# aantoine890/navierstokes

Hardware: AMD Instinct MI355X
Metric: fp64 CSR SpMV GFLOP/s & % HBM roofline @ nnz; 1/2/4/8 GPU (higher is better)
Workload: dtype f64

## Files before the change

include/mi355_spmv.h:

```cpp
#ifndef MI355_SPMV_H
#define MI355_SPMV_H

#ifdef __cplusplus
extern "C" {
#endif

#define MI355_SPMV_VERSION 501

enum {
    MI_OK = 0,
    MI_ERR_ARG = 1,
    MI_ERR_NODEVICE = 2,
    MI_ERR_HIP = 3,
    MI_ERR_ALLOC = 4,
    MI_ERR_UNSUPPORTED = 5,
    MI_ERR_STATE = 6
};

#define MI_MAX_POWERS 16

typedef struct mi_csr_s* mi_csr_t;
typedef struct mi_bcsr4_s* mi_bcsr4_t;
typedef struct mi_part_s* mi_part_t;
typedef void* mi_stream_t;

enum {
    MI_KERNEL_AUTO = 0,
    MI_KERNEL_STREAM = 1,
    MI_KERNEL_RING = 2,
    MI_KERNEL_ROWPAR = 3,
    MI_KERNEL_BCSR4 = 4,
    MI_KERNEL_MRING = 6,
    MI_KERNEL_SSTREAM = 7,
    MI_KERNEL_TILE = 5
};

int mi_version(void);
const char* mi_strerror(int status);
const char* mi_last_error(void);
int mi_device_count(int* count);
int mi_set_device(int device);
int mi_device_synchronize(void);
int mi_flush_cache(void);
int mi_flush_cache_async(mi_stream_t s);

int mi_csr_create(int n, int ncols, const int* ptrow, const int* indcol, const double* coef, mi_csr_t* out);
int mi_csr_create_mapped(int n, int ncols, const int* ptrow, const int* indcol, const double* coef,
                         const int* rowmap, mi_csr_t* out);
int mi_csr_destroy(mi_csr_t A);
int mi_csr_update_values(mi_csr_t A, const double* coef);
int mi_csr_update_values_dev(mi_csr_t A, const double* d_coef, mi_stream_t s);
int mi_csr_dims(mi_csr_t A, int* n, int* ncols, long long* nnz);
int mi_csr_reorder_info(mi_csr_t A, int* reordered, int* block, double* spread_before, double* spread_after,
                        double* us_natural, double* us_reordered);
int mi_csr_perm(mi_csr_t A, int* reordered, int* perm );
int mi_vec_to_internal_dev(mi_csr_t A, const double* d_x, double* d_x_int, mi_stream_t s);
int mi_vec_from_internal_dev(mi_csr_t A, const double* d_x_int, double* d_x, mi_stream_t s);
int mi_spmv_internal_dev(mi_csr_t A, const double* d_x_int, double* d_y_int, mi_stream_t s);
int mi_spmk_internal_dev(mi_csr_t A, int k, const double* d_x_int, double* const* d_y_int_out, mi_stream_t s);
int mi_reorder_probe(int n, const int* ptrow, const int* indcol, int* block, int* perm, double* spread_before,
                     double* spread_after);
int mi_csr_set_kernel(mi_csr_t A, int kernel_id);
int mi_csr_ring_info(mi_csr_t A, int* config_id, int* runs, int* runs_not_ringable, double* nnz_fraction_ringable);
int mi_csr_ring_shape_info(mi_csr_t A, int* blocks, int* lean, int* depth, double* us_aligned, double* us_unaligned);
int mi_csr_tune_info(mi_csr_t A, double* us_ring, double* us_stream);
int mi_csr_tune_detail(mi_csr_t A, double us[5], int* ring_nt, int* stream_nt);
int mi_ring_plan_probe(int n, const int* ptrow, const int* indcol, int config_id, int* nblk, int* runs,
                       int* runs_not_ringable, double* nnz_fraction_ringable, int* max_slot);
int mi_csr_tile_info(mi_csr_t A, int* built, int* nblk, double* unique_per_nnz, double us[2], int* nt);
int mi_tile_plan_probe(int n, const int* ptrow, const int* indcol, int threads, int* nblk, long long* distinct_total,
                       int* max_distinct, long long* nnz_listed);
int mi_csr_placement_info(mi_csr_t A, int* n_values, int* n_total, double* us, int cap);
int mi_vec_alloc_placed(mi_csr_t A, int nvec, int draws, double** d_vecs, double* us, int cap, int* n_us);
int mi_vec_free_placed(double* d_vec);
int mi_csr_sstream_info(mi_csr_t A, int* built, int* rounds, long long* steps, double* padding, double us[4], int* form);
int mi_sstream_plan_probe(int n, int ncols, const int* ptrow, const int* indcol, int* eligible, int* rounds, long long* steps, double* padding);
int mi_sstream_plan_probe_ex(int n, int ncols, const int* ptrow, const int* indcol, int shift, int ghost_lo, int ghost_hi, int* eligible, int* rounds,
                             long long* steps, double* padding, int* ghost_workgroups, int* rounds_min_max);
int mi_sstream_mw_plan_probe(int n, int ncols, const int* ptrow, const int* indcol, int shift, int* eligible, int* rounds, long long* steps, double* padding);
int mi_csr_mring_info(mi_csr_t A, int* built, int* runs, int* runs_not_served, double* nnz_fraction_served, double us[2], int* nt);
int mi_mring_plan_probe(int n, const int* ptrow, const int* indcol, int* nblk, int* runs, int* runs_not_served,
                        double* nnz_fraction_served, long long* window_restarts);
int mi_mring_plan_deal_probe(int n, const int* ptrow, const int* indcol, int* table_len, int* run_blocks, int cap);
int mi_ring_plan_lean(int n, const int* ptrow, const int* indcol, int config_id, int* lean);
#define MI_RING_CENSUS_LEN 62
int mi_ring_plan_census(int n, const int* ptrow, const int* indcol, int config_id, long long* counters, int cap);
#define MI_MRING_CENSUS_LEN 43
// ... 248 lines not shown
```

navierstokes_amd/csrc/capi_blas1.hip:

```cpp
#include "capi_internal.hpp"
#include "blas1_kernels.hpp"
#include "blas1_multi.hpp"
#include "gmres_kernels.hpp"

static std::map<std::pair<int, hipStream_t>, double*> g_ws;
constexpr size_t kWsMdot = 4 * (size_t)kMaxPartials;
constexpr size_t kWsDots2 = kWsMdot + (size_t)kMultiMax * kMaxPartials;
constexpr size_t kWsDoubles = kWsDots2 + kMultiMax + 8;

int get_ws(hipStream_t s, double** out)
{
    int dev = 0;
    HIP_TRY(hipGetDevice(&dev));
    std::lock_guard<std::mutex> lock(g_mu);
    double*& w = g_ws[std::make_pair(dev, s)];
    if (!w) HIP_TRY(hipMalloc(&w, sizeof(double) * kWsDoubles));
    *out = w;
    return MI_OK;
}

static bool blas1_nt(int n)
{
    static const int forced = getenv("MI355_BLAS1_NT") ? atoi(getenv("MI355_BLAS1_NT")) : -1;
    return forced >= 0 ? forced != 0 : n >= kBlas1NtMin;
}

static int red_geometry(int n, int* np, int* seg)
{
    long long s = ((long long)n + kMaxPartials - 1) / kMaxPartials;
    const int q = 2 * kRedWG;
    s = ((s + q - 1) / q) * q;
    if (s < q) s = q;
    *seg = (int)s;
    *np = (int)(((long long)n + s - 1) / s);
    if (*np < 1) *np = 1;
    return MI_OK;
// ... 565 lines not shown
    HIP_TRY(hipMemcpy(dots, dd, sizeof(double) * (size_t)m, hipMemcpyDeviceToHost));
    return MI_OK;
}

extern "C" int mi_maxpy(int n, int m, const double* coef, int negate, const double* const* basis, double* y)
{
    int rc = multi_check(n, m, basis, y);
    if (rc) return rc;
    CHECK_ARG(m == 0 || coef, "null coefficients");
    if ((rc = need_device())) return rc;
    if (m == 0 || n == 0) return MI_OK;
    Scratch S;
    std::vector<const double*> dv((size_t)m);
    double *dy = nullptr, *dc = nullptr;
    for (int j = 0; j < m; j++) {
        double* p = nullptr;
        if ((rc = S.up(basis[j], n, &p))) return rc;
        dv[j] = p;
    }
    if ((rc = S.up(y, n, &dy)) || (rc = S.up(coef, m, &dc))) return rc;
    if ((rc = mi_maxpy_dev(n, m, dc, negate, dv.data(), dy, nullptr, nullptr))) return rc;
    HIP_TRY(hipMemcpy(y, dy, sizeof(double) * (size_t)n, hipMemcpyDeviceToHost));
    return MI_OK;
}

int gather_perm(mi_csr_t A, const double* d_x, double* d_xp, hipStream_t s)
{
    if (A->reorder_block == 4 && (((uintptr_t)d_x | (uintptr_t)d_xp) & 15) == 0) {
        const int nn = A->n / 4;
        hipLaunchKernelGGL(gather_nodes_kernel, dim3(launch_grid(nn, 256, 4096)), dim3(256), 0, s, nn, A->d_iperm, d_x, d_xp);
        HIP_TRY(hipGetLastError());
        return MI_OK;
    }
    return mi_gather_dev(A->n, A->d_iperm, d_x, d_xp, (mi_stream_t)s);
}


__global__ __launch_bounds__(256) void scatter_kernel(int m, const int* __restrict__ idx, const double* __restrict__ src,
                                                      double* __restrict__ dst)
{
    const long long stride = (long long)gridDim.x * blockDim.x;
    for (long long i = (long long)blockIdx.x * blockDim.x + threadIdx.x; i < m; i += stride) dst[idx[i]] = src[i];
}

int scatter_perm(mi_csr_t A, const double* d_src, double* d_dst, hipStream_t s)
{
    hipLaunchKernelGGL(scatter_kernel, dim3(launch_grid(A->n, 256, 2048)), dim3(256), 0, s, A->n, A->d_iperm, d_src, d_dst);
    HIP_TRY(hipGetLastError());
    return MI_OK;
}
```

navierstokes_amd/csrc/capi_csr.hip:

```cpp
#include "capi_internal.hpp"
#include "reorder.hpp"
#include "mring_plan.hpp"
#include "tile_plan.hpp"

int get_table(mi_csr_t A, int nnzb, BlockTable** out)
{
    auto it = A->tables.find(nnzb);
    if (it == A->tables.end()) {
        std::vector<int> rows, ptrs;
        int row_align = A->nnz < 20000000 ? 64 : 1;
        if (const char* e = getenv("MI355_STREAM_ROW_ALIGN")) row_align = std::max(1, atoi(e));
        build_row_blocks(A->n, A->h_ptrow.data(), nnzb, 4 * kWG, rows, ptrs, row_align, 7);
        BlockTable T;
        T.nnzb = nnzb;
        T.nblk = (int)rows.size() - 1;
        std::vector<int2> h(rows.size());
        for (size_t i = 0; i < rows.size(); i++) h[i] = make_int2(rows[i], ptrs[i]);
        HIP_TRY(T.d_blk.upload(h));
        it = A->tables.emplace(nnzb, std::move(T)).first;
    }
    *out = &it->second;
    return MI_OK;
}

// ... 591 lines not shown
                    const int* rowmap, mi_csr_t* out, int ghost_lo, int ghost_hi, bool defer_placement)
{
    CHECK_ARG(out, "out is null");
    *out = nullptr;
    CsrInput in{n, ncols, ptrow, indcol, coef, rowmap, ghost_lo, ghost_hi};
    int rc = check_input(in);
    if (rc || (rc = need_device())) return rc;
    std::unique_ptr<mi_csr_s> owner(new (std::nothrow) mi_csr_s());
    mi_csr_t A = owner.get();
    if (!A) return fail(MI_ERR_ALLOC, "host allocation failed");
    A->n = n;
    A->ncols = ncols;
    A->nnz = in.nnz;
    A->ghost_lo = ghost_lo;
    A->ghost_hi = ghost_hi;
    A->h_ptrow.assign(ptrow, ptrow + n + 1);
    if ((rc = upload(A, in)) || (rc = plan_ring(A, in)) || (rc = plan_optional(A, in)) || (rc = attach_blocked(A, in))) return rc;
    load_defaults(A, in);
    const bool forced_kernel = apply_forced_kernel(A);
    if (!forced_kernel && in.nnz < kMeasureNnz && A->auto_kernel == MI_KERNEL_RING && !in.ghosts()) A->auto_kernel = MI_KERNEL_STREAM;
    if (!forced_kernel && !env_is("MI355_SPMV_AUTOTUNE", "0") && in.nnz >= kMeasureNnz && (rc = measure_at_create(A, in, defer_placement))) return rc;
    HIP_TRY(hipStreamSynchronize(nullptr));
    *out = owner.release();
    return MI_OK;
}

static int time_handle(mi_csr_t A, int warm, int timed, double* us)
{
    LaunchTimer tm;
    ScratchPair sp;
    int rc = sp.alloc((size_t)(A->ncols > 0 ? A->ncols : 1), (size_t)(A->n_out > 0 ? A->n_out : 1));
    if (rc || (rc = tm.init())) return rc;
    return time_on(tm, A, sp.x, sp.y, warm, timed, us);
}

static int maybe_reorder(mi_csr_t A, const int* ptrow, const int* indcol, const double* coef)
{
    const bool force = env_is("MI355_REORDER", "1");
    if (env_is("MI355_REORDER", "0")) return MI_OK;
    const int n = A->n;
    if (A->mapped || n != A->ncols || n < 8 || A->nnz == 0) return MI_OK;
    if (!force && (n < 100000 || resolve_kernel(A) == MI_KERNEL_RING || resolve_kernel(A) == MI_KERNEL_SSTREAM)) return MI_OK;
    const int block = csr_has_block4_pattern(n, ptrow, indcol) ? 4 : 1;
    const double nn = (double)n / block;
    const double spread = mean_column_distance(n, ptrow, indcol, block);
    A->spread_before = spread;
    if (!force && spread < 2.0 * std::pow(nn, 2.0 / 3.0)) return MI_OK;
    Reorder R;
    rcm_reorder(n, ptrow, indcol, block, R);
    A->reorder_block = block;
    A->spread_after = R.spread_after;
    if (!force && R.spread_after > 0.5 * spread) return MI_OK;
    std::vector<int> p2, c2, src_start;
    std::vector<double> v2;
    permute_csr(n, ptrow, indcol, coef, R, p2, c2, v2, src_start);
    mi_csr_t inner = nullptr;
    int rc = csr_create_impl(n, n, p2.data(), c2.data(), v2.data(), R.iperm.data(), &inner);
    if (rc) return rc;
    A->inner.reset(inner);
    HIP_TRY(A->d_iperm.alloc((size_t)n));
    HIP_TRY(A->d_src_start.alloc((size_t)n));
    HIP_TRY(A->d_xp.alloc((size_t)n));
    HIP_TRY(A->d_iperm.fill(R.iperm));
    HIP_TRY(A->d_src_start.fill(src_start));
    bool keep = true;
    if (!force && !env_is("MI355_SPMV_AUTOTUNE", "0")) {
        const int timed = A->nnz < 40000000 ? 12 : 6;
        (void)A->inner.own.release();
        rc = time_handle(A, 3, timed, &A->us_natural);
        A->inner.reset(inner);
        if (rc) return rc;
        if ((rc = time_handle(A, 3, timed, &A->us_reordered))) return rc;
        keep = A->us_reordered < 0.97 * A->us_natural;
    }
    if (!keep) {
        A->inner.reset(), A->d_iperm = {}, A->d_src_start = {}, A->d_xp = {};
        return MI_OK;
    }
    A->h_iperm = R.iperm;
    A->xp_claimed = false;
    A->d_ptrow = {}, A->d_indcol = {}, A->d_coef = {};
    A->drop_tables();
    A->ring = {}, A->tile = {}, A->mring = {}, A->ss = {}, A->blocked.reset();
    return MI_OK;
}

extern "C" int mi_csr_create(int n, int ncols, const int* ptrow, const int* indcol, const double* coef, mi_csr_t* out)
{
    int rc = csr_create_impl(n, ncols, ptrow, indcol, coef, nullptr, out, 0, 0, true);
    if (rc) return rc;
    if ((rc = maybe_reorder(*out, ptrow, indcol, coef)) || (!(*out)->inner && (rc = placement_draws(*out, nullptr, n == ncols))) ||
        (hipStreamSynchronize(nullptr) != hipSuccess && (rc = fail(MI_ERR_HIP, "mi_csr_create: synchronize")))) {
        mi_csr_destroy(*out);
        *out = nullptr;
    }
    return rc;
}

extern "C" int mi_reorder_probe(int n, const int* ptrow, const int* indcol, int* block, int* perm, double* spread_before,
                                double* spread_after)
{
    CHECK_ARG(n >= 0 && ptrow && (ptrow[n] == 0 || indcol), "bad argument");
    for (int i = 0; i < n; i++) {
        CHECK_ARG(ptrow[i] <= ptrow[i + 1], "ptrow must be non-decreasing");
        for (int k = ptrow[i]; k < ptrow[i + 1]; k++) CHECK_ARG(indcol[k] >= 0 && indcol[k] < n, "column index outside [0, n)");
    }
    const int b = csr_has_block4_pattern(n, ptrow, indcol) ? 4 : 1;
    Reorder R;
    rcm_reorder(n, ptrow, indcol, b, R);
    if (block) *block = b;
    if (perm)
        for (int i = 0; i < n; i++) perm[i] = R.perm[i];
    if (spread_before) *spread_before = R.spread_before;
    if (spread_after) *spread_after = R.spread_after;
    return MI_OK;
}

extern "C" int mi_csr_reorder_info(mi_csr_t A, int* reordered, int* block, double* spread_before, double* spread_after,
                                   double* us_natural, double* us_reordered)
{
    CHECK_ARG(A, "null handle");
    if (reordered) *reordered = A->inner ? 1 : 0;
    if (block) *block = A->reorder_block;
    if (spread_before) *spread_before = A->spread_before;
    if (spread_after) *spread_after = A->spread_after;
    if (us_natural) *us_natural = A->us_natural;
    if (us_reordered) *us_reordered = A->us_reordered;
    return MI_OK;
}

extern "C" int mi_csr_perm(mi_csr_t A, int* reordered, int* perm)
{
    CHECK_ARG(A, "null handle");
    if (reordered) *reordered = A->inner ? 1 : 0;
    if (perm) {
        if (A->inner) {
            CHECK_ARG((int)A->h_iperm.size() == A->n, "permutation not kept on this handle");
            for (int r = 0; r < A->n; r++) perm[A->h_iperm[r]] = r;
        } else {
            for (int i = 0; i < A->n; i++) perm[i] = i;
        }
    }
    return MI_OK;
}

extern "C" int mi_vec_to_internal_dev(mi_csr_t A, const double* d_x, double* d_x_int, mi_stream_t s)
{
    CHECK_ARG(A, "null handle");
    if (A->n == 0) return MI_OK;
    CHECK_ARG(d_x && d_x_int && d_x != d_x_int, "null vector, or in place");
    if (A->inner) return gather_perm(A, d_x, d_x_int, (hipStream_t)s);
    HIP_TRY(hipMemcpyAsync(d_x_int, d_x, sizeof(double) * (size_t)A->n, hipMemcpyDeviceToDevice, (hipStream_t)s));
    return MI_OK;
}

extern "C" int mi_vec_from_internal_dev(mi_csr_t A, const double* d_x_int, double* d_x, mi_stream_t s)
{
    CHECK_ARG(A, "null handle");
    if (A->n == 0) return MI_OK;
    CHECK_ARG(d_x && d_x_int && d_x != d_x_int, "null vector, or in place");
// ... 835 lines not shown
```

navierstokes_amd/csrc/capi_internal.hpp:

```cpp
#pragma once
#include "mi355_spmv.h"

#include <hip/hip_runtime.h>

#include <cstdio>
#include <cstdlib>
#include <cmath>
#include <chrono>
#include <cstring>
#include <map>
#include <memory>
#include <mutex>
#include <new>
#include <string>
#include <vector>

#include "dev_array.hpp"
#include "dispatch.hpp"
#include "partition.hpp"
#include "push_exchange.hpp"
#include "ring_plan.hpp"
#include "spmv_kernels.hpp"
#include "spmv_ring.hpp"
#include "spmv_sstream_mw.hpp"

using namespace mi355;

extern thread_local std::string g_err;

static inline int fail(int code, const std::string& msg)
{
    g_err = msg;
    return code;
}

static inline int hip_fail(hipError_t e, const char* what)
{
    const int code = (e == hipErrorNoDevice || e == hipErrorInvalidDevice || e == hipErrorInsufficientDriver) ? MI_ERR_NODEVICE
                                                                                                               : (e == hipErrorOutOfMemory ? MI_ERR_ALLOC : MI_ERR_HIP);
    return fail(code, std::string(what) + ": " + hipGetErrorString(e));
}

#define HIP_TRY_AS(what, expr)                            \
    do {                                                  \
        hipError_t e_ = (expr);                           \
        if (e_ != hipSuccess) return hip_fail(e_, what);  \
    } while (0)
#define HIP_TRY(expr) HIP_TRY_AS(#expr, expr)

#define CHECK_ARG(cond, msg)                        \
    do {                                            \
        if (!(cond)) return fail(MI_ERR_ARG, msg);  \
// ... 102 lines not shown
    DevArray<int> d_rng;
    DevArray<unsigned short> d_slots;
    bool nt = false, skew = false;
};

struct TileTable {
    int nblk = 0;
    DevArray<int> d_desc;
    DevArray<unsigned> d_ulist;
    DevArray<unsigned short> d_slots;
    double unique_per_nnz = 0.0;
    bool nt = false;
    bool skew = false;
};

struct SstreamCopy {
    bool mw = false;
    SsDevice dev;
    int nwg = 0, rounds = 0;
    int shift = 0;
    long long steps = 0;
    double padding = 0.0;
    int max_slice_nnz = 0;
    bool nt = true;
    bool deep = true;
    bool fusable = false;
    bool asked = false;
    std::vector<int> h_wg_halo;
    std::vector<SsWg> h_wg;
};
struct SstreamTable : SstreamCopy {
    double tune_us[4] = {0, 0, 0, 0};
    SstreamCopy& copy() { return *this; }
};

template <class H, class Destroy = std::default_delete<H>>
struct OwnedHandle {
    std::unique_ptr<H, Destroy> own;
    operator H*() const { return own.get(); }
    H* operator->() const { return own.get(); }
    void reset(H* p = nullptr) { own.reset(p); }
};

struct DevPowers {
    std::vector<DevArray<double>> own;
    std::vector<double*> ptr;
    int grow(int k, size_t n)
    {
        while ((int)own.size() < k) {
            DevArray<double> a;
            HIP_TRY(a.alloc(n));
            ptr.push_back(a);
            own.push_back(std::move(a));
        }
        return MI_OK;
    }
    void release()
    {
        for (auto& a : own) a = {};
        own.clear(), ptr.clear();
    }
};

struct SpmkTables {
    DevArray<unsigned> flags;
    DevArray<int> dep_ptr, dep_run;
// ... 64 lines not shown
    RingTable ring;
    TileTable tile;
    SstreamTable ss;
    MringTable mring;
    int kernel = MI_KERNEL_AUTO;
    int auto_kernel = MI_KERNEL_STREAM;
    std::vector<double> place_us;
    int place_draws_coef = 0;
    DevArray<double> kept_x, kept_y;
    double tune_us[MI_KERNEL_SSTREAM + 1][2] = {};
    double tune_us_ring_aligned = 0.0, tune_us_ring_unaligned = 0.0;
    bool stream_nt = false;
    OwnedHandle<mi_bcsr4_s> blocked;
    int n_out = 0;
    OwnedHandle<mi_csr_s> inner;
    DevArray<int> d_iperm;
    std::vector<int> h_iperm;
    DevArray<int> d_src_start;
    DevArray<double> d_xp;
    hipStream_t xp_stream = nullptr;
    bool xp_claimed = false;
    std::map<hipStream_t, DevArray<double>> xp_more;
    DevPowers d_pp;
    DevArray<double> d_vtmp;
    double spread_before = 0.0, spread_after = 0.0, us_natural = 0.0, us_reordered = 0.0;
    int reorder_block = 0;
    DevArray<double> d_x, d_y;
    DevPowers d_pow;
    SpmkTables kstep;
    unsigned kstep_epoch = 0;
    int kstep_setup = 0;
    int kstep_choice[9] = {0, 0, 0, 0, 0, 0, 0, 0, 0};
    double kstep_us[9][2] = {};
    void drop_tables()
    {
        for (auto& kv : tables) kv.second = {};
        tables.clear();
    }
    ~mi_csr_s()
    {
        d_ptrow = {}, d_indcol = {}, d_coef = {}, d_rowmap = {}, d_x = {}, d_y = {}, kept_x = {}, kept_y = {}, d_pow.release();
        drop_tables();
        ring = {}, tile = {}, mring = {}, ss = {}, blocked.reset(), inner.reset(), d_iperm = {}, d_src_start = {}, d_xp = {};
        for (auto& kv : xp_more) kv.second = {};
        d_vtmp = {}, d_pp.release(), kstep = {};
    }
};

struct RcclCommDestroy { void operator()(void* comm) const; };
struct IpcMappingClose { void operator()(void* base) const; };
struct WinRegistryErase { void operator()(std::string* key) const; };
using RcclComm = std::unique_ptr<void, RcclCommDestroy>;
using IpcMappings = std::vector<std::unique_ptr<void, IpcMappingClose>>;
using WinRegistryEntry = std::unique_ptr<std::string, WinRegistryErase>;

struct PartRccl {
    RcclComm comm;
    OwnedStream comm_stream;
    OwnedEvent ev_pack, ev_comm;
    DevArray<double> d_sendbuf;
    unsigned step_no = 0;
    bool flag_handoff = false;
};

struct PartAllGather {
    DevArray<int> d_ag_idx;
    DevArray<int> d_ag_src;
    DevArray<double> d_ag_send;
    DevArray<double> d_ag_recv;
    int ag_slice = 0;
    bool ready() const { return d_ag_idx != nullptr; }
};

struct PushWindow {
    IpcMappings ipc_opened;
    WinRegistryEntry win_entry;
    DevArray<char> win;
    unsigned* win_flags = nullptr;
// ... 53 lines not shown

static inline size_t win_data_offset(int nranks) { return ((size_t)nranks * kWinFlagStride * sizeof(unsigned) + 255) / 256 * 256; }

extern std::mutex g_mu;
int get_ws(hipStream_t s, double** out);

struct Scratch {
    std::vector<DevArray<double>> bufs;
    ~Scratch()
    {
        for (auto& a : bufs) a = {};
    }
    int up(const double* h, size_t n, double** d)
    {
        *d = nullptr;
        DevArray<double> a;
        int rc = dev_alloc(a, n, 1);
        if (rc) return rc;
        *d = a;
        bufs.push_back(std::move(a));
        if (h && n) HIP_TRY(hipMemcpy(*d, h, sizeof(double) * n, hipMemcpyHostToDevice));
        return MI_OK;
    }
};

int csr_create_impl(int n, int ncols, const int* ptrow, const int* indcol, const double* coef, const int* rowmap, mi_csr_t* out,
                    int ghost_lo = 0, int ghost_hi = 0, bool defer_placement = false);
int resolve_kernel(const mi_csr_s* A);
int get_table(mi_csr_t A, int nnzb, BlockTable** out);
int launch_spmv(mi_csr_t A, const double* d_x, double* d_y, hipStream_t s, bool use_map = true, const RingComm* comm = nullptr,
                const RingDot* dot = nullptr);
bool ring_dot_eligible(const mi_csr_s* A);
int reorder_scratch(mi_csr_t A, hipStream_t s, double** buf);
void launch_ring_cfg(const mi_csr_s* A, const CsrView& V, const double* d_x, double* d_y, hipStream_t s, const RingComm* comm, const RingDot* dot);
int spmk_unmapped(mi_csr_t H, int k, const double* d_x, double* const* d_y, hipStream_t s);
int gather_perm(mi_csr_t A, const double* d_x, double* d_xp, hipStream_t s);
int ortho_update_from_parts(int n, int nparts, const double* parts, double alpha, const double* d_b, const double* d_x1, double* d_x3, double* d_beta_out,
                            hipStream_t s);
int scatter_perm(mi_csr_t A, const double* d_src, double* d_dst, hipStream_t s);
int residual_norm_dev(int n, const double* d_b, const double* d_w, double* d_r, double* d_out, hipStream_t s);
constexpr size_t kLdsBytesPerCU = 160 * 1024;
static inline size_t spmm_tile_lds(const SpmmTilePlan* T, int s) { return T ? (size_t)T->umax * (4 * s + 2) * sizeof(double) : (size_t)-1; }
hipError_t spmm_tile_launch(const mi_bcsr4_s* A, const SpmmTilePlan* Pl, const Bcsr4View& V, int s, int arith, const double* X, long long ldx,
                            double* Y, long long ldy, hipStream_t st);
hipError_t spmm_otile_launch(const mi_bcsr4_s* A, const SpmmTilePlan* Pl, const Bcsr4View& V, int s, int arith, bool nt, const double* X, long long ldx,
                             double* Y, long long ldy, hipStream_t st);
int part_push_window(mi_part_s* P);
void part_push_layout(const mi_part_s* P, long long* layout );
int part_push_connect_bases(mi_part_s* P, void* const* bases , const long long* layouts,
                            IpcMappings opened = {}, bool peer_on_my_device = false);
int part_ext_launch(mi_part_s* P, const double* d_x_ext, double* d_y_local, unsigned step, unsigned spin_max, hipStream_t s, unsigned long long* trace, int* grid_out);
int launch_sstream(mi_csr_t A, const double* d_x, double* d_y, const int* rowmap, hipStream_t s, const RingComm* comm = nullptr);
static inline bool sstream_y_ok(const mi_csr_s* A, const double* yy, const int* map) { return map || A->ss.mw || (((uintptr_t)(yy - A->ss.shift)) & 15) == 0; }
int bcsr4_values_changed(mi_bcsr4_s* A, hipStream_t s);
void bcsr4_drop_sliced(mi_bcsr4_s* A);
int bcsr4_refresh_from_csr(mi_bcsr4_s* A, const int* d_csr_ptrow, const double* d_src, double* d_csr_out, hipStream_t s);
int launch_bcsr4(mi_bcsr4_t A, const double* d_x, double* d_y, mi_stream_t s, bool use_map);
struct Bilu4Apply {
    bool sweeps, f32;
    int sf, sb;
};
int bilu4_apply_prepare(mi_bilu4_t F, const Bilu4Apply& how);
int bilu4_apply_dev(mi_bilu4_t F, const Bilu4Apply& how, const double* d_b, double* d_x, hipStream_t s);
```

navierstokes_amd/csrc/launch_csr.hip:

```cpp
#include "capi_internal.hpp"
#include "spmv_rowpar.hpp"
#include "spmv_tile.hpp"
#include "spmv_mring.hpp"

int reorder_scratch(mi_csr_t A, hipStream_t s, double** buf)
{
    std::lock_guard<std::mutex> lock(g_mu);
    if (!A->xp_claimed || A->xp_stream == s) {
        A->xp_claimed = true;
        A->xp_stream = s;
        *buf = A->d_xp;
        return MI_OK;
    }
    DevArray<double>& b = A->xp_more[s];
    if (!b) {
        if (stream_is_capturing(s)) return fail(MI_ERR_STATE, "first product of a relabelled handle on this stream: run one outside stream capture first (it allocates a gather buffer)");
        HIP_TRY(b.alloc((size_t)A->n));
    }
    *buf = b;
    return MI_OK;
}

bool ring_dot_eligible(const mi_csr_s* A)
{
    if (A->inner || A->n == 0 || A->d_rowmap || A->y_offset) return false;
    if (resolve_kernel(A) != MI_KERNEL_RING) return false;
    const RingTable& R = A->ring;
    int depth = R.cfg.depth;
    if (const char* e = getenv("MI355_RING_DEPTH")) depth = atoi(e);
    return R.cfg.id == 4 && R.lean && depth != 3 && R.all_in_loop && R.wgs >= 1 && R.wgs <= 1024  &&
           !env_is("MI355_SPMV_DOT_EPILOGUE", "0");
}

int launch_spmv(mi_csr_t A, const double* d_x, double* d_y, hipStream_t s, bool use_map, const RingComm* comm, const RingDot* dot)
{
    if (dot && !ring_dot_eligible(A)) return fail(MI_ERR_STATE, "dot epilogue requested on a handle whose launch cannot carry it");
    if (A->n == 0) return MI_OK;
    const bool ss_fused = comm && resolve_kernel(A) == MI_KERNEL_SSTREAM && A->ss.fusable;
    if (comm && (A->inner || A->d_rowmap || (resolve_kernel(A) != MI_KERNEL_RING && !ss_fused)))
        return fail(MI_ERR_STATE, "fused multi-GPU step: the combined piece must be an unmapped, unreordered handle served by the ring or the sliced-stream kernel");
    if (A->inner) {
        double* xp = nullptr;
        int rc = reorder_scratch(A, s, &xp);
        if (rc) return rc;
        if ((rc = gather_perm(A, d_x, xp, s))) return rc;
        return launch_spmv(A->inner, xp, d_y, s, true);
    }
    int kid = resolve_kernel(A);
    if (kid == MI_KERNEL_SSTREAM && !dot && (!comm || ss_fused)) {
        const int* map = use_map ? A->d_rowmap : nullptr;
        double* yy = d_y + (use_map ? A->y_offset : 0);
        if (sstream_y_ok(A, yy, map)) return launch_sstream(A, d_x, yy, map, s, comm);
        if (comm) return fail(MI_ERR_ARG, "fused multi-GPU step: y must be 16-byte aligned");
        kid = A->ring.d_plan && A->ring.ok_fraction >= 0.90 ? MI_KERNEL_RING : MI_KERNEL_STREAM;
    } else if (kid == MI_KERNEL_SSTREAM) {
        kid = A->ring.d_plan && A->ring.ok_fraction >= 0.90 ? MI_KERNEL_RING : MI_KERNEL_STREAM;
    }
    if (use_map) d_y += A->y_offset;
    CsrView V{};
    V.n = A->n;
    V.ncols = A->ncols;
    V.ptrow = A->d_ptrow;
    V.indcol = A->d_indcol;
    V.coef = A->d_coef;
    V.rowmap = use_map ? A->d_rowmap : nullptr;
    V.blk = nullptr;
    V.blk_span = nullptr;
    V.nblk = 0;
    if (kid == MI_KERNEL_BCSR4 && (((uintptr_t)d_x) & 15) == 0) return launch_bcsr4(A->blocked, d_x, d_y, (mi_stream_t)s, use_map);
    if (kid == MI_KERNEL_BCSR4) {
        BlockTable* T = nullptr;
        int rc = get_table(A, 1024, &T);
        if (rc) return rc;
        V.blk = T->d_blk;
        V.nblk = T->nblk;
        const int grid = kNXCD * ((T->nblk + kNXCD - 1) / kNXCD);
        hipLaunchKernelGGL((spmv_csr_stream<1024, false>), dim3(grid), dim3(kWG), 0, s, V, d_x, d_y);
        HIP_TRY(hipGetLastError());
// ... 40 lines not shown
```

navierstokes_amd/mpk.py:

```python
from __future__ import annotations

import ctypes
import os

import numpy as np

_HERE = os.path.dirname(os.path.abspath(__file__))
LIB_PATH = os.environ.get("MI355_SPMV_LIBRARY") or os.path.join(_HERE, "csrc", "libmi355spmv.so")

MI_OK = 0
KERNEL_AUTO, KERNEL_STREAM, KERNEL_RING, KERNEL_ROWPAR = 0, 1, 2, 3
KERNELS = {"auto": 0, "stream": 1, "ring": 2, "rowpar": 3, "bcsr4": 4, "tile": 5, "mring": 6, "sstream": 7}

_c = ctypes
_vp = ctypes.c_void_p
_LIB = None


class MiError(RuntimeError):
    def __init__(self, status, detail):
        super().__init__(f"libmi355spmv status {status}: {detail}")
        self.status = status


# ... 26 lines not shown
        "mi_flush_cache": [],
        "mi_flush_cache_async": [_vp],
        "mi_csr_create": [i, i, _vp, _vp, _vp, P(_vp)],
        "mi_csr_create_mapped": [i, i, _vp, _vp, _vp, _vp, P(_vp)],
        "mi_csr_destroy": [_vp],
        "mi_csr_update_values": [_vp, _vp],
        "mi_csr_update_values_dev": [_vp, _vp, _vp],
        "mi_bcsr4_update_values": [_vp, _vp],
        "mi_bcsr4_update_values_dev": [_vp, _vp, _vp],
        "mi_orthonormalize_against_basis": [i, i, _vp, _vp, _vp],
        "mi_orthonormalize_against_basis_dev": [i, i, _vp, _vp, _vp, _vp],
        "mi_mdot": [i, i, _vp, _vp, _vp],
        "mi_mdot_dev": [i, i, _vp, _vp, _vp, _vp],
        "mi_maxpy": [i, i, _vp, i, _vp, _vp],
        "mi_maxpy_dev": [i, i, _vp, i, _vp, _vp, _vp, _vp],
        "mi_cgs_dev": [i, i, _vp, _vp, i, _vp, _vp, _vp],
        "mi_part_status": [_vp],
        "mi_part_push_export": [_vp, _vp, _vp],
        "mi_part_push_connect": [_vp, _vp, _vp],
        "mi_part_spmv_push_dev": [_vp, _vp, _vp, _vp],
        "mi_part_push_info": [_vp, P(i), P(i), P(i)],
        "mi_part_sends_contiguous": [_vp, P(i)],
        "mi_part_combined_info": [_vp, P(i)],
        "mi_part_push_disable": [_vp],
        "mi_part_push_unfuse": [_vp],
        "mi_bcsr4_spmm": [_vp, i, _vp, ll, _vp, ll, i],
        "mi_bcsr4_spmm_info": [_vp, i, P(i), P(i), P(i), P(d)],
        "mi_bcsr4_spmm_dev": [_vp, i, _vp, ll, _vp, ll, i, _vp],
        "mi_spmm_dev": [_vp, i, _vp, ll, _vp, ll, _vp],
        "mi_krylov_basis_dev": [_vp, i, _vp, _vp, ll, i, _vp, _vp],
        "mi_krylov_basis_cgs_dev": [_vp, i, _vp, _vp, ll, i, _vp, _vp],
        "mi_csr_reorder_info": [_vp, P(i), P(i), P(d), P(d), P(d), P(d)],
        "mi_reorder_probe": [i, _vp, _vp, P(i), _vp, P(d), P(d)],
        "mi_csr_perm": [_vp, P(i), _vp],
        "mi_vec_to_internal_dev": [_vp, _vp, _vp, _vp],
        "mi_vec_from_internal_dev": [_vp, _vp, _vp, _vp],
        "mi_spmv_internal_dev": [_vp, _vp, _vp, _vp],
        "mi_spmk_internal_dev": [_vp, i, _vp, _vp, _vp],
        "mi_csr_dims": [_vp, P(i), P(i), P(ll)],
        "mi_csr_set_kernel": [_vp, i],
        "mi_csr_get_kernel": [_vp, P(i)],
        "mi_csr_ring_info": [_vp, P(i), P(i), P(i), P(d)],
        "mi_csr_ring_shape_info": [_vp, P(i), P(i), P(i), P(d), P(d)],
        "mi_csr_tune_info": [_vp, P(d), P(d)],
        "mi_csr_tune_detail": [_vp, P(d), P(_c.c_int), P(_c.c_int)],
        "mi_csr_set_nontemporal": [_vp, i, i],
        "mi_csr_block4_structure": [i, _vp, _vp, P(i), P(_c.c_longlong)],
        "mi_ring_plan_probe": [i, _vp, _vp, i, P(i), P(i), P(i), P(d), P(i)],
        "mi_ring_plan_lean": [i, _vp, _vp, i, P(i)],
        "mi_ring_plan_census": [i, _vp, _vp, i, _vp, i],
        "mi_mring_plan_census": [i, _vp, _vp, _vp, i],
        "mi_csr_tile_info": [_vp, P(i), P(i), P(d), P(d), P(i)],
        "mi_bcsr4_tile_info": [_vp, P(i), P(i), P(d), P(d)],
        "mi_bcsr4_sell_info": [_vp, P(i), P(i), P(ll), P(d), P(d)],
        "mi_bcsr4_sell_plan_probe": [i, _vp, _vp, i, P(i), P(ll), P(i), _vp, _vp, _vp],
        "mi_bcsr4_spmm_plan_probe": [i, _vp, _vp, i, i, P(i), P(i), P(i), P(d), _vp, ll, _vp, ll, _vp, ll, _vp, ll],
        "mi_csr_mring_info": [_vp, P(i), P(i), P(i), P(d), P(d), P(i)],
        "mi_csr_sstream_info": [_vp, P(i), P(i), P(ll), P(d), P(d), P(i)],
        "mi_sstream_plan_probe": [i, i, _vp, _vp, P(i), P(i), P(ll), P(d)],
        "mi_sstream_plan_probe_ex": [i, i, _vp, _vp, i, i, i, P(i), P(i), P(ll), P(d), P(i), P(i)],
        "mi_sstream_mw_plan_probe": [i, i, _vp, _vp, i, P(i), P(i), P(ll), P(d)],
        "mi_csr_placement_info": [_vp, P(i), P(i), P(d), i],
        "mi_vec_alloc_placed": [_vp, i, i, P(_vp), P(d), i, P(i)],
        "mi_vec_free_placed": [_vp],
        "mi_mring_plan_deal_probe": [i, _vp, _vp, P(i), _vp, i],
        "mi_mring_plan_probe": [i, _vp, _vp, P(i), P(i), P(i), P(d), P(ll)],
# ... 292 lines not shown
        return out, [round(us[k], 2) for k in range(nus.value)]

    def mring_info(self):
        b, r, bad, nt = _c.c_int(), _c.c_int(), _c.c_int(), _c.c_int()
        f = _c.c_double()
        us = (_c.c_double * 2)()
        check(lib().mi_csr_mring_info(self.handle, _c.byref(b), _c.byref(r), _c.byref(bad), _c.byref(f), us, _c.byref(nt)))
        return dict(built=bool(b.value), runs=r.value, runs_not_served=bad.value, nnz_fraction=f.value, us=us[0], us_nt=us[1],
                    nt=bool(nt.value))

    def sstream_info(self):
        b, r, fm = _c.c_int(), _c.c_int(), _c.c_int()
        st = _c.c_longlong()
        pad = _c.c_double()
        us = (_c.c_double * 4)()
        check(lib().mi_csr_sstream_info(self.handle, _c.byref(b), _c.byref(r), _c.byref(st), _c.byref(pad), us, _c.byref(fm)))
        return dict(built=bool(b.value), rounds=r.value, steps=st.value, padding=pad.value, us_d8_nt=us[0], us_d8_temporal=us[1], us_d12_nt=us[2],
                    us_d12_temporal=us[3], form=fm.value)

    def tile_info(self):
        b, nb, nt = _c.c_int(), _c.c_int(), _c.c_int()
        u = _c.c_double()
        us = (_c.c_double * 2)()
        check(lib().mi_csr_tile_info(self.handle, _c.byref(b), _c.byref(nb), _c.byref(u), us, _c.byref(nt)))
        return dict(built=bool(b.value), nblk=nb.value, unique_per_nnz=u.value, us=us[0], us_nt=us[1], nt=bool(nt.value))

    def reorder_info(self):
        r, b = _c.c_int(), _c.c_int()
        v = [_c.c_double() for _ in range(4)]
        check(lib().mi_csr_reorder_info(self.handle, _c.byref(r), _c.byref(b), *[_c.byref(t) for t in v]))
        return dict(reordered=bool(r.value), block=b.value, spread_before=v[0].value, spread_after=v[1].value,
                    us_natural=v[2].value, us_reordered=v[3].value)

    def spmk_info(self, k):
        e, o = _c.c_int(), _c.c_int()
        a, b = _c.c_double(), _c.c_double()
        check(lib().mi_csr_spmk_info(self.handle, int(k), _c.byref(e), _c.byref(o), _c.byref(a), _c.byref(b)))
        return dict(eligible=bool(e.value), one_launch=bool(o.value), us_k_launches=a.value, us_one_launch=b.value)

    def dot_in_epilogue(self):
        r = _c.c_int()
        check(lib().mi_csr_dot_epilogue_info(self.handle, _c.byref(r)))
        return bool(r.value)

    def dot_epilogue_layout(self):
        t, w, nb = _c.c_int(), _c.c_int(), _c.c_int()
        check(lib().mi_csr_dot_epilogue_layout(self.handle, _c.byref(t), _c.byref(w), _c.byref(nb), None, None, None, 0, 0))
        first = np.zeros(w.value + 1, np.int32)
        row0 = np.zeros(max(nb.value, 1), np.int32)
        rows = np.zeros(max(nb.value, 1), np.int32)
        check(lib().mi_csr_dot_epilogue_layout(self.handle, _c.byref(t), _c.byref(w), _c.byref(nb), first.ctypes.data,
                                               row0.ctypes.data, rows.ctypes.data, first.size, row0.size))
        return dict(threads=t.value, run_first_block=first, block_row0=row0[: nb.value], block_rows=rows[: nb.value])

    def perm(self):
        r = _c.c_int()
        p = np.empty(self.n, np.int32)
        check(lib().mi_csr_perm(self.handle, _c.byref(r), p.ctypes.data))
        return bool(r.value), p

    def to_internal(self, x, out=None):
        import torch
        out = torch.empty_like(x) if out is None else out
        check(lib().mi_vec_to_internal_dev(self.handle, _dev_ptr(x, self.n, "x"), _dev_ptr(out, self.n, "x_int"), _stream_ptr()))
        return out

# ... 1146 lines not shown
```

Measured before the change: 1245.

## Add two-pass LDS-tiled permutation for reordered SpMV gather and scatter

Adds a tiled two-pass permutation. Each block loads a contiguous source tile into LDS and writes the entries bucketed by destination tile, then a second pass reads each bucket and places entries through LDS into contiguous output. This replaces the random single-pass gather and scatter for relabelled handles. At creation time the handle times single-pass against tiled forms for the x gather and y scatter and keeps whichever wins by a margin. It costs an extra intermediate buffer, plan tables and two kernel launches per permutation, and adds autotune time at creation.

Result: slower. 1226 (-1.5%).

```diff
diff --git a/include/mi355_spmv.h b/include/mi355_spmv.h
--- a/include/mi355_spmv.h
+++ b/include/mi355_spmv.h
@@ -53,6 +53,11 @@
 int mi_csr_dims(mi_csr_t A, int* n, int* ncols, long long* nnz);
 int mi_csr_reorder_info(mi_csr_t A, int* reordered, int* block, double* spread_before, double* spread_after,
                         double* us_natural, double* us_reordered);
+int mi_csr_perm_form_info(mi_csr_t A, int* x_form, int* y_form, double* us , int* tile , int* tiles ,
+                          long long* table_bytes, long long* scratch_bytes);
+int mi_csr_set_perm_form(mi_csr_t A, int x_form, int y_form);
+int mi_perm_tiles_probe(int n, const int* p, int tile, int* ts, int* td, unsigned short* srcloc, unsigned* tpos, unsigned short* dstloc,
+                        long long* runs, double* amplification, const char** violation);
 int mi_csr_perm(mi_csr_t A, int* reordered, int* perm );
 int mi_vec_to_internal_dev(mi_csr_t A, const double* d_x, double* d_x_int, mi_stream_t s);
 int mi_vec_from_internal_dev(mi_csr_t A, const double* d_x_int, double* d_x, mi_stream_t s);
diff --git a/navierstokes_amd/csrc/capi_blas1.hip b/navierstokes_amd/csrc/capi_blas1.hip
--- a/navierstokes_amd/csrc/capi_blas1.hip
+++ b/navierstokes_amd/csrc/capi_blas1.hip
@@ -2,6 +2,7 @@
 #include "blas1_kernels.hpp"
 #include "blas1_multi.hpp"
 #include "gmres_kernels.hpp"
+#include "perm_tiles.hpp"
 
 static std::map<std::pair<int, hipStream_t>, double*> g_ws;
 constexpr size_t kWsMdot = 4 * (size_t)kMaxPartials;
@@ -633,7 +634,25 @@
         HIP_TRY(hipGetLastError());
         return MI_OK;
     }
+    if (A->perm_form(0) == 1)
+        if (double* scratch = reorder_scratch_peek(A, s)) return perm_tiles_run(A->pt_gather, A->n, d_x, scratch + A->perm_pad(), d_xp, s);
     return mi_gather_dev(A->n, A->d_iperm, d_x, d_xp, (mi_stream_t)s);
+}
+
+int perm_tiles_prepare()
+{
+    HIP_TRY(hipFuncSetAttribute(reinterpret_cast<const void*>(perm_tiles_pass_a), hipFuncAttributeMaxDynamicSharedMemorySize, (int)kLdsBytesPerCU));
+    HIP_TRY(hipFuncSetAttribute(reinterpret_cast<const void*>(perm_tiles_pass_b), hipFuncAttributeMaxDynamicSharedMemorySize, (int)kLdsBytesPerCU));
+    return MI_OK;
+}
+
+int perm_tiles_run(const PermTilesTable& T, int n, const double* d_src, double* d_t, double* d_dst, hipStream_t s)
+{
+    hipLaunchKernelGGL(perm_tiles_pass_a, dim3((unsigned)T.nsrc), dim3(kPermTileThreads), sizeof(double) * (size_t)T.ts, s, n, T.ts, T.srcloc.get(), d_src, d_t);
+    hipLaunchKernelGGL(perm_tiles_pass_b, dim3((unsigned)T.ndst), dim3(kPermTileThreads), sizeof(double) * (size_t)T.td, s, n, T.td, T.tpos.get(), T.dstloc.get(),
+                       d_t, d_dst);
+    HIP_TRY(hipGetLastError());
+    return MI_OK;
 }
 
 
@@ -646,6 +665,8 @@
 
 int scatter_perm(mi_csr_t A, const double* d_src, double* d_dst, hipStream_t s)
 {
+    if (A->perm_form(0) == 1)
+        if (double* scratch = reorder_scratch_peek(A, s)) return perm_tiles_run(A->pt_scatter, A->n, d_src, scratch + A->perm_pad(), d_dst, s);
     hipLaunchKernelGGL(scatter_kernel, dim3(launch_grid(A->n, 256, 2048)), dim3(256), 0, s, A->n, A->d_iperm, d_src, d_dst);
     HIP_TRY(hipGetLastError());
     return MI_OK;
diff --git a/navierstokes_amd/csrc/capi_csr.hip b/navierstokes_amd/csrc/capi_csr.hip
--- a/navierstokes_amd/csrc/capi_csr.hip
+++ b/navierstokes_amd/csrc/capi_csr.hip
@@ -647,6 +647,61 @@
     int rc = sp.alloc((size_t)(A->ncols > 0 ? A->ncols : 1), (size_t)(A->n_out > 0 ? A->n_out : 1));
     if (rc || (rc = tm.init())) return rc;
     return time_on(tm, A, sp.x, sp.y, warm, timed, us);
+}
+
+static bool perm_tiles_race_wanted(const mi_csr_s* A)
+{
+    return (size_t)A->n * 8 > ((size_t)4 << 20) && !env_is("MI355_SPMV_AUTOTUNE", "0") && !getenv("MI355_PERM_TILED");
+}
+
+static int upload_perm_tiles(PermTilesTable& T, int n, const std::vector<int>& p, int tile)
+{
+    PermTilesPlan P;
+    build_perm_tiles_plan(n, p.data(), tile, tile, P);
+    PermTilesTable L;
+    L.ts = P.ts, L.td = P.td, L.nsrc = P.nsrc, L.ndst = P.ndst;
+    int rc;
+    if ((rc = dev_upload(L.srcloc, P.srcloc)) || (rc = dev_upload(L.tpos, P.tpos)) || (rc = dev_upload(L.dstloc, P.dstloc))) return rc;
+    T = std::move(L);
+    return MI_OK;
+}
+
+static int plan_perm_tiles(mi_csr_t A, const Reorder& R)
+{
+    const char* te = getenv("MI355_PERM_TILE");
+    if (A->reorder_block != 1 || env_is("MI355_PERM_TILED", "0")) return MI_OK;
+    if (!env_is("MI355_PERM_TILED", "1") && !te && !perm_tiles_race_wanted(A)) return MI_OK;
+    const int tile = perm_tile_size(A->n, te ? std::max(1, atoi(te)) : 0);
+    PermTilesTable g, sc;
+    int rc;
+    if ((rc = perm_tiles_prepare()) || (rc = upload_perm_tiles(g, A->n, R.iperm, tile)) || (rc = upload_perm_tiles(sc, A->n, R.perm, tile))) return rc;
+    A->pt_gather = std::move(g), A->pt_scatter = std::move(sc);
+    A->d_xp = {};
+    HIP_TRY(A->d_xp.alloc(A->scratch_len()));
+    if (env_is("MI355_PERM_TILED", "1")) A->perm_form_measured[0] = A->perm_form_measured[1] = 1;
+    return MI_OK;
+}
+
+static int race_perm_forms(mi_csr_t A)
+{
+    if (!A->pt_gather.srcloc || !perm_tiles_race_wanted(A)) return MI_OK;
+    LaunchTimer tm;
+    ScratchPair sp;
+    int rc = sp.alloc((size_t)A->n, (size_t)A->n);
+    if (rc || (rc = tm.init())) return rc;
+    const int timed = A->nnz < 40000000 ? 12 : 6;
+    double* us = A->perm_us;
+    auto run = [&](int xf, int yf, double* out) {
+        A->perm_form_measured[0] = xf, A->perm_form_measured[1] = yf;
+        return time_on(tm, A, sp.x, sp.y, 3, timed, out);
+    };
+    if ((rc = run(0, 0, &us[0])) || (rc = run(1, 0, &us[1]))) return rc;
+    const int xf = us[1] < 0.97 * us[0];
+    us[2] = us[xf];
+    if ((rc = run(xf, 1, &us[3]))) return rc;
+    A->perm_form_measured[0] = xf;
+    A->perm_form_measured[1] = us[3] < 0.97 * us[2];
+    return MI_OK;
 }
 
 static int maybe_reorder(mi_csr_t A, const int* ptrow, const int* indcol, const double* coef)
@@ -693,6 +748,7 @@
         return MI_OK;
     }
     A->h_iperm = R.iperm;
+    if ((rc = plan_perm_tiles(A, R)) || (rc = race_perm_forms(A))) return rc;
     A->xp_claimed = false;
     A->d_ptrow = {}, A->d_indcol = {}, A->d_coef = {};
     A->drop_tables();
@@ -741,6 +797,55 @@
     if (spread_after) *spread_after = A->spread_after;
     if (us_natural) *us_natural = A->us_natural;
     if (us_reordered) *us_reordered = A->us_reordered;
+    return MI_OK;
+}
+
+extern "C" int mi_csr_perm_form_info(mi_csr_t A, int* x_form, int* y_form, double* us, int* tile, int* tiles, long long* table_bytes,
+                                     long long* scratch_bytes)
+{
+    CHECK_ARG(A, "null handle");
+    const PermTilesTable& G = A->pt_gather;
+    if (x_form) *x_form = A->perm_form(0);
+    if (y_form) *y_form = A->perm_form(1);
+    if (us)
+        for (int i = 0; i < 4; i++) us[i] = A->perm_us[i];
+    if (tile) tile[0] = G.ts, tile[1] = G.td;
+    if (tiles) tiles[0] = G.nsrc, tiles[1] = G.ndst;
+    if (table_bytes) *table_bytes = G.srcloc ? 2LL * 8 * (long long)A->perm_pad() : 0;
+    if (scratch_bytes) *scratch_bytes = A->inner ? 8LL * (long long)A->scratch_len() : 0;
+    return MI_OK;
+}
+
+extern "C" int mi_csr_set_perm_form(mi_csr_t A, int x_form, int y_form)
+{
+    CHECK_ARG(A, "null handle");
+    CHECK_ARG(x_form >= -1 && x_form <= 1 && y_form >= -1 && y_form <= 1, "a form is 0 (one pass), 1 (tiled) or -1 (as measured)");
+    if (!A->pt_gather.srcloc) return fail(MI_ERR_STATE, "the handle has no tiled permutation plan (not relabelled, relabelled by nodes, or too small: MI355_PERM_TILE)");
+    A->perm_form_set[0] = x_form;
+    A->perm_form_set[1] = y_form;
+    return MI_OK;
+}
+
+extern "C" int mi_perm_tiles_probe(int n, const int* p, int tile, int* ts, int* td, unsigned short* srcloc, unsigned* tpos, unsigned short* dstloc,
+                                   long long* runs, double* amplification, const char** violation)
+{
+    CHECK_ARG(n >= 0 && (n == 0 || p) && tile >= 0, "bad argument");
+    std::vector<char> seen((size_t)n, 0);
+    for (int i = 0; i < n; i++) {
+        CHECK_ARG(p[i] >= 0 && p[i] < n && !seen[(size_t)p[i]], "p is not a permutation of 0 .. n-1");
+        seen[(size_t)p[i]] = 1;
+    }
+    const int sz = perm_tile_size(n, tile);
+    PermTilesPlan P;
+    build_perm_tiles_plan(n, p, sz, sz, P);
+    if (ts) *ts = sz;
+    if (td) *td = sz;
+    if (srcloc) std::copy(P.srcloc.begin(), P.srcloc.end(), srcloc);
+    if (tpos) std::copy(P.tpos.begin(), P.tpos.end(), tpos);
+    if (dstloc) std::copy(P.dstloc.begin(), P.dstloc.end(), dstloc);
+    if (runs) *runs = P.runs;
+    if (amplification) *amplification = perm_tiles_read_amplification(P);
+    if (violation) *violation = check_perm_tiles_plan(P, n, p);
     return MI_OK;
 }
 
diff --git a/navierstokes_amd/csrc/capi_internal.hpp b/navierstokes_amd/csrc/capi_internal.hpp
--- a/navierstokes_amd/csrc/capi_internal.hpp
+++ b/navierstokes_amd/csrc/capi_internal.hpp
@@ -18,6 +18,7 @@
 #include "dev_array.hpp"
 #include "dispatch.hpp"
 #include "partition.hpp"
+#include "perm_tiles_plan.hpp"
 #include "push_exchange.hpp"
 #include "ring_plan.hpp"
 #include "spmv_kernels.hpp"
@@ -186,6 +187,13 @@
 struct SstreamTable : SstreamCopy {
     double tune_us[4] = {0, 0, 0, 0};
     SstreamCopy& copy() { return *this; }
+};
+
+struct PermTilesTable {
+    int ts = 0, td = 0, nsrc = 0, ndst = 0;
+    DevArray<unsigned short> srcloc;
+    DevArray<unsigned> tpos;
+    DevArray<unsigned short> dstloc;
 };
 
 template <class H, class Destroy = std::default_delete<H>>
@@ -316,6 +324,13 @@
     int kstep_setup = 0;
     int kstep_choice[9] = {0, 0, 0, 0, 0, 0, 0, 0, 0};
     double kstep_us[9][2] = {};
+    PermTilesTable pt_gather, pt_scatter;
+    int perm_form_measured[2] = {0, 0};
+    int perm_form_set[2] = {-1, -1};
+    double perm_us[4] = {0, 0, 0, 0};
+    int perm_form(int side) const { return !pt_gather.srcloc ? 0 : perm_form_set[side] >= 0 ? perm_form_set[side] : perm_form_measured[side]; }
+    size_t perm_pad() const { return ((size_t)n + kPermTileAlign - 1) / kPermTileAlign * kPermTileAlign; }
+    size_t scratch_len() const { return pt_gather.srcloc ? 3 * perm_pad() : (size_t)n; }
     void drop_tables()
     {
         for (auto& kv : tables) kv.second = {};
@@ -327,7 +342,7 @@
         drop_tables();
         ring = {}, tile = {}, mring = {}, ss = {}, blocked.reset(), inner.reset(), d_iperm = {}, d_src_start = {}, d_xp = {};
         for (auto& kv : xp_more) kv.second = {};
-        d_vtmp = {}, d_pp.release(), kstep = {};
+        d_vtmp = {}, d_pp.release(), kstep = {}, pt_gather = {}, pt_scatter = {};
     }
 };
 
@@ -447,12 +462,15 @@
                 const RingDot* dot = nullptr);
 bool ring_dot_eligible(const mi_csr_s* A);
 int reorder_scratch(mi_csr_t A, hipStream_t s, double** buf);
+double* reorder_scratch_peek(mi_csr_t A, hipStream_t s);
 void launch_ring_cfg(const mi_csr_s* A, const CsrView& V, const double* d_x, double* d_y, hipStream_t s, const RingComm* comm, const RingDot* dot);
 int spmk_unmapped(mi_csr_t H, int k, const double* d_x, double* const* d_y, hipStream_t s);
 int gather_perm(mi_csr_t A, const double* d_x, double* d_xp, hipStream_t s);
 int ortho_update_from_parts(int n, int nparts, const double* parts, double alpha, const double* d_b, const double* d_x1, double* d_x3, double* d_beta_out,
                             hipStream_t s);
 int scatter_perm(mi_csr_t A, const double* d_src, double* d_dst, hipStream_t s);
+int perm_tiles_prepare();
+int perm_tiles_run(const PermTilesTable& T, int n, const double* d_src, double* d_t, double* d_dst, hipStream_t s);
 int residual_norm_dev(int n, const double* d_b, const double* d_w, double* d_r, double* d_out, hipStream_t s);
 constexpr size_t kLdsBytesPerCU = 160 * 1024;
 static inline size_t spmm_tile_lds(const SpmmTilePlan* T, int s) { return T ? (size_t)T->umax * (4 * s + 2) * sizeof(double) : (size_t)-1; }
diff --git a/navierstokes_amd/csrc/launch_csr.hip b/navierstokes_amd/csrc/launch_csr.hip
--- a/navierstokes_amd/csrc/launch_csr.hip
+++ b/navierstokes_amd/csrc/launch_csr.hip
@@ -15,10 +15,18 @@
     DevArray<double>& b = A->xp_more[s];
     if (!b) {
         if (stream_is_capturing(s)) return fail(MI_ERR_STATE, "first product of a relabelled handle on this stream: run one outside stream capture first (it allocates a gather buffer)");
-        HIP_TRY(b.alloc((size_t)A->n));
+        HIP_TRY(b.alloc(A->scratch_len()));
     }
     *buf = b;
     return MI_OK;
+}
+
+double* reorder_scratch_peek(mi_csr_t A, hipStream_t s)
+{
+    std::lock_guard<std::mutex> lock(g_mu);
+    if (A->xp_claimed && A->xp_stream == s) return A->d_xp;
+    auto it = A->xp_more.find(s);
+    return it != A->xp_more.end() ? it->second.get() : nullptr;
 }
 
 bool ring_dot_eligible(const mi_csr_s* A)
@@ -44,6 +52,11 @@
         int rc = reorder_scratch(A, s, &xp);
         if (rc) return rc;
         if ((rc = gather_perm(A, d_x, xp, s))) return rc;
+        if (A->perm_form(1) == 1) {
+            double* ys = xp + 2 * A->perm_pad();
+            if ((rc = launch_spmv(A->inner, xp, ys, s, false))) return rc;
+            return perm_tiles_run(A->pt_scatter, A->n, ys, xp + A->perm_pad(), d_y, s);
+        }
         return launch_spmv(A->inner, xp, d_y, s, true);
     }
     int kid = resolve_kernel(A);
diff --git a/navierstokes_amd/csrc/perm_tiles.hpp b/navierstokes_amd/csrc/perm_tiles.hpp
--- /dev/null
+++ b/navierstokes_amd/csrc/perm_tiles.hpp
@@ -0,0 +1,43 @@
+#pragma once
+#include <hip/hip_runtime.h>
+
+#include "perm_tiles_plan.hpp"
+
+namespace mi355 {
+
+constexpr int kPermTileThreads = 1024;
+
+static __global__ __launch_bounds__(kPermTileThreads) void perm_tiles_pass_a(int n, int ts, const unsigned short* __restrict__ srcloc,
+                                                                             const double* __restrict__ src, double* __restrict__ t)
+{
+    extern __shared__ double perm_lds[];
+    const long long lo = (long long)blockIdx.x * ts;
+    const int cnt = (int)(n - lo < ts ? n - lo : ts);
+    for (int j = threadIdx.x; j < cnt; j += kPermTileThreads) perm_lds[j] = src[lo + j];
+    __syncthreads();
+    const unsigned* loc2 = reinterpret_cast<const unsigned*>(srcloc + lo);
+    double2* t2 = reinterpret_cast<double2*>(t + lo);
+    const int pairs = (cnt + 1) >> 1;
+    for (int q = threadIdx.x; q < pairs; q += kPermTileThreads) {
+        const unsigned w = loc2[q];
+        double2 v;
+        v.x = perm_lds[w & 0xffffu];
+        v.y = perm_lds[w >> 16];
+        t2[q] = v;
+    }
+}
+
+static __global__ __launch_bounds__(kPermTileThreads) void perm_tiles_pass_b(int n, int td, const unsigned* __restrict__ tpos,
+                                                                             const unsigned short* __restrict__ dstloc, const double* __restrict__ t,
+                                                                             double* __restrict__ dst)
+{
+    extern __shared__ double perm_lds[];
+    const long long lo = (long long)blockIdx.x * td;
+    const int cnt = (int)(n - lo < td ? n - lo : td);
+#pragma unroll 4
+    for (int j = threadIdx.x; j < cnt; j += kPermTileThreads) perm_lds[dstloc[lo + j]] = t[tpos[lo + j]];
+    __syncthreads();
+    for (int j = threadIdx.x; j < cnt; j += kPermTileThreads) dst[lo + j] = perm_lds[j];
+}
+
+}
diff --git a/navierstokes_amd/csrc/perm_tiles_plan.hpp b/navierstokes_amd/csrc/perm_tiles_plan.hpp
--- /dev/null
+++ b/navierstokes_amd/csrc/perm_tiles_plan.hpp
@@ -0,0 +1,129 @@
+#pragma once
+#include <algorithm>
+#include <cstdint>
+#include <vector>
+
+namespace mi355 {
+
+constexpr int kPermTileDefault = 16384;
+constexpr int kPermTileMax = 20000;
+constexpr int kPermTileMin = 64;
+constexpr int kPermTileAlign = 16;
+constexpr int kPermTileCus = 256;
+
+struct PermTilesPlan {
+    int n = 0;
+    int ts = 0, td = 0;
+    int nsrc = 0, ndst = 0;
+    std::vector<unsigned short> srcloc;
+    std::vector<unsigned> tpos;
+    std::vector<unsigned short> dstloc;
+    long long runs = 0;
+};
+
+inline int perm_tile_size(long long n, int forced = 0)
+{
+    if (forced > 0) return std::max(kPermTileMin, std::min(kPermTileDefault, forced)) / kPermTileAlign * kPermTileAlign;
+    if (n <= kPermTileDefault) return kPermTileDefault;
+    const long long rounds = (n + (long long)kPermTileCus * kPermTileMax - 1) / ((long long)kPermTileCus * kPermTileMax);
+    const long long tiles = rounds * kPermTileCus;
+    const long long tile = ((n + tiles - 1) / tiles + kPermTileAlign - 1) / kPermTileAlign * kPermTileAlign;
+    return (int)std::min<long long>(tile, kPermTileMax);
+}
+
+inline void build_perm_tiles_plan(int n, const int* p, int ts, int td, PermTilesPlan& out)
+{
+    out = PermTilesPlan();
+    out.n = n;
+    out.ts = ts;
+    out.td = td;
+    if (n <= 0) return;
+    const int nsrc = (n + ts - 1) / ts, ndst = (n + td - 1) / td;
+    out.nsrc = nsrc;
+    out.ndst = ndst;
+    const size_t padded = ((size_t)n + kPermTileAlign - 1) / kPermTileAlign * kPermTileAlign;
+    out.srcloc.assign(padded, 0);
+    out.tpos.assign(padded, 0);
+    out.dstloc.assign(padded, 0);
+    std::vector<long long> at((size_t)nsrc * ndst + 1, 0);
+    for (int i = 0; i < n; i++) at[(size_t)(p[i] / ts) * ndst + i / td + 1]++;
+    for (size_t q = 1; q < at.size(); q++) {
+        out.runs += at[q] != 0;
+        at[q] += at[q - 1];
+    }
+    std::vector<long long> bt((size_t)nsrc * ndst, 0);
+    for (int d = 0; d < ndst; d++) {
+        long long j = (long long)d * td;
+        for (int s = 0; s < nsrc; s++) {
+            const size_t q = (size_t)s * ndst + d;
+            bt[q] = j;
+            j += at[q + 1] - at[q];
+        }
+    }
+    for (int i = 0; i < n; i++) {
+        const size_t q = (size_t)(p[i] / ts) * ndst + i / td;
+        const long long k = at[q]++, j = bt[q]++;
+        out.srcloc[(size_t)k] = (unsigned short)(p[i] % ts);
+        out.tpos[(size_t)j] = (unsigned)k;
+        out.dstloc[(size_t)j] = (unsigned short)(i % td);
+    }
+}
+
+inline const char* check_perm_tiles_plan(const PermTilesPlan& P, int n, const int* p)
+{
+    if (P.n != n) return "plan built for another n";
+    if (n <= 0) return nullptr;
+    if (P.ts < kPermTileAlign || P.td < kPermTileAlign || P.ts % kPermTileAlign || P.td % kPermTileAlign || P.ts > 65536 || P.td > 65536)
+        return "tile size not a multiple of the line, or beyond a 16-bit position";
+    if (P.nsrc != (n + P.ts - 1) / P.ts || P.ndst != (n + P.td - 1) / P.td) return "tile counts do not cover n";
+    const size_t padded = ((size_t)n + kPermTileAlign - 1) / kPermTileAlign * kPermTileAlign;
+    if (P.srcloc.size() != padded || P.tpos.size() != padded || P.dstloc.size() != padded) return "table length is not n rounded up to the line";
+    std::vector<int> t((size_t)n, -1), dst((size_t)n, -1);
+    std::vector<unsigned char> hit((size_t)n, 0);
+    for (int s = 0; s < P.nsrc; s++) {
+        const long long lo = (long long)s * P.ts;
+        const int cnt = (int)std::min<long long>(P.ts, n - lo);
+        for (long long k = lo; k < lo + cnt; k++) {
+            if (P.srcloc[(size_t)k] >= cnt) return "srcloc outside its source tile";
+            t[(size_t)k] = (int)(lo + P.srcloc[(size_t)k]);
+        }
+    }
+    for (size_t k = (size_t)n; k < padded; k++)
+        if (P.srcloc[k] != 0 || P.tpos[k] != 0 || P.dstloc[k] != 0) return "padding entry not zero";
+    for (int d = 0; d < P.ndst; d++) {
+        const long long lo = (long long)d * P.td;
+        const int cnt = (int)std::min<long long>(P.td, n - lo);
+        for (long long j = lo; j < lo + cnt; j++) {
+            const unsigned k = P.tpos[(size_t)j];
+            if (k >= (unsigned)n) return "tpos outside t";
+            if (hit[k]) return "tpos names an entry of t twice";
+            hit[k] = 1;
+            if (P.dstloc[(size_t)j] >= cnt) return "dstloc outside its destination tile";
+            int& o = dst[(size_t)(lo + P.dstloc[(size_t)j])];
+            if (o != -1) return "two entries placed at one destination";
+            o = t[k];
+            if (j > lo && t[k] / P.ts < t[P.tpos[(size_t)j - 1]] / P.ts) return "a destination tile's entries are not ordered by source tile";
+        }
+    }
+    for (int i = 0; i < n; i++)
+        if (dst[(size_t)i] != p[i]) return "replay does not give src[p[i]]";
+    return nullptr;
+}
+
+inline double perm_tiles_read_amplification(const PermTilesPlan& P)
+{
+    if (P.n <= 0) return 1.0;
+    long long sectors = 0;
+    for (int d = 0; d < P.ndst; d++) {
+        const long long lo = (long long)d * P.td, hi = std::min<long long>(lo + P.td, P.n);
+        long long last = -1;
+        for (long long j = lo; j < hi; j++) {
+            const long long sec = (long long)P.tpos[(size_t)j] / 8;
+            sectors += sec != last;
+            last = sec;
+        }
+    }
+    return (double)sectors / ((double)P.n / 8.0);
+}
+
+}
diff --git a/navierstokes_amd/mpk.py b/navierstokes_amd/mpk.py
--- a/navierstokes_amd/mpk.py
+++ b/navierstokes_amd/mpk.py
@@ -82,6 +82,9 @@
         "mi_krylov_basis_cgs_dev": [_vp, i, _vp, _vp, ll, i, _vp, _vp],
         "mi_csr_reorder_info": [_vp, P(i), P(i), P(d), P(d), P(d), P(d)],
         "mi_reorder_probe": [i, _vp, _vp, P(i), _vp, P(d), P(d)],
+        "mi_csr_perm_form_info": [_vp, P(i), P(i), _vp, _vp, _vp, P(ll), P(ll)],
+        "mi_csr_set_perm_form": [_vp, i, i],
+        "mi_perm_tiles_probe": [i, _vp, i, P(i), P(i), _vp, _vp, _vp, P(ll), P(d), P(_c.c_char_p)],
         "mi_csr_perm": [_vp, P(i), _vp],
         "mi_vec_to_internal_dev": [_vp, _vp, _vp, _vp],
         "mi_vec_from_internal_dev": [_vp, _vp, _vp, _vp],
@@ -440,6 +443,18 @@
         return dict(reordered=bool(r.value), block=b.value, spread_before=v[0].value, spread_after=v[1].value,
                     us_natural=v[2].value, us_reordered=v[3].value)
 
+    def perm_form_info(self):
+        xf, yf = _c.c_int(), _c.c_int()
+        us = (_c.c_double * 4)()
+        tile, tiles = (_c.c_int * 2)(), (_c.c_int * 2)()
+        tb, sb = _c.c_longlong(), _c.c_longlong()
+        check(lib().mi_csr_perm_form_info(self.handle, _c.byref(xf), _c.byref(yf), us, tile, tiles, _c.byref(tb), _c.byref(sb)))
+        return dict(x_form=xf.value, y_form=yf.value, us_x_single=us[0], us_x_tiled=us[1], us_y_mapped=us[2], us_y_tiled=us[3],
+                    tile_src=tile[0], tile_dst=tile[1], tiles_src=tiles[0], tiles_dst=tiles[1], table_bytes=tb.value, scratch_bytes=sb.value)
+
+    def set_perm_form(self, x_form, y_form):
+        check(lib().mi_csr_set_perm_form(self.handle, int(x_form), int(y_form)))
+
     def spmk_info(self, k):
         e, o = _c.c_int(), _c.c_int()
         a, b = _c.c_double(), _c.c_double()
```
